# erincatto/solver2d

Measured on NVIDIA B200. Metric: constraint_iters_per_sec, higher is better.
Workload: dtype f32

## Files before the change

include/s2b_device.h:

```cpp
#pragma once

#include <stddef.h>
#include <stdint.h>

#ifdef __cplusplus
extern "C"
{
#endif

typedef struct s2bWorld s2bWorld;

#if defined(__GNUC__)
	#define S2B_API __attribute__((visibility("default")))
#else
	#define S2B_API
#endif


#define S2B_ROW_VALID 0x1
#define S2B_BODY_ADD_FORCE 0x8

typedef struct s2bBodyRow
{
	int32_t index;
// ... 104 lines not shown
};

typedef struct s2bCounters
{
	int32_t bodyCapacity, shapeCapacity, jointCapacity;
	int32_t contactCount;
	int32_t constraintCount;
	int32_t jointCount;
	int32_t groupCount;
	int32_t overflowCount;
	int32_t treeHeight;
	int32_t movedCount;
	int32_t pairPassCount;
	int32_t kernelLaunches;
	int32_t graphReplays;
	int32_t graphCaptures;
	int64_t scratchBytes;
	int32_t regionCount;
	int32_t cutCount;
	int32_t cutGroupCount;
	int32_t recolouredCount;
	int32_t largeLeafCount;
	int32_t pairRebuildCount;
} s2bCounters;


S2B_API s2bWorld* s2b_world_create(int cudaDevice, int solverType);
S2B_API void s2b_world_destroy(s2bWorld* world);

S2B_API void s2b_set_gravity(s2bWorld* world, float gx, float gy);
S2B_API void s2b_set_schedule(s2bWorld* world, int schedule);
S2B_API void s2b_set_max_colors(s2bWorld* world, int maxColors);
S2B_API void s2b_set_persistent(s2bWorld* world, int enable);
S2B_API void s2b_set_warm_gather(s2bWorld* world, int enable);
S2B_API void s2b_set_graph(s2bWorld* world, int enable);
S2B_API void s2b_set_regions(s2bWorld* world, int mode);
S2B_API void s2b_set_dataflow(s2bWorld* world, int enable);


S2B_API void s2b_upload_bodies(s2bWorld* world, const s2bBodyRow* rows, int count, int bodyCapacity);
S2B_API void s2b_upload_shapes(s2bWorld* world, const s2bShapeRow* rows, int count, int shapeCapacity);
S2B_API void s2b_upload_joints(s2bWorld* world, const s2bJointRow* rows, int count, int jointCapacity);
S2B_API void s2b_upload_contacts(s2bWorld* world, const s2bContactRow* rows, int count);
S2B_API void s2b_upload_joint_pairs(s2bWorld* world, const uint64_t* blockKeys, int blockCount, const uint64_t* destroyKeys,
									int destroyCount);
typedef struct s2bForceRow
// ... 57 lines not shown
```

solver2d_b200/csrc/device/broadphase.cu:

```cuda
#include "s2b_internal.cuh"

#include <cub/cub.cuh>
#include <thrust/iterator/counting_iterator.h>

#include <algorithm>

struct BroadScratch
{
	DevArray<int> validFlag;
	DevArray<int> leafShape;
	DevArray<unsigned> mortonIn, mortonOut;
	DevArray<int> leafIn, leafOut;
	DevArray<int> sortedShape;
	DevArray<int> counters;
	DevArray<int> boundsBits;
	DevArray<float4> nodeBox;
	DevArray<int> movedShapes;
	DevArray<int> movedFlag;
	DevArray<int> largeShapes;
	DevArray<unsigned long long> newKey;
	DevArray<int2> newShapes;
	DevArray<int> keepFlag, keepSlots;
	DevArray<unsigned long long> mergeKeyIn, mergeKeyOut;
	DevArray<int> mergeSrcIn, mergeSrcOut;
	DevArray<char> cubTemp;
	int newPairCap = 0;
	bool treeValid = false;
	int treeShapeCap = 0;
	int treeReuses = 0;
	DevArray<unsigned long long> pairHash;
	unsigned long long hashMask = 0;
	unsigned long long hashVersion = ~0ull;
	bool prefetched = false;
	bool lastPassRan = false;
	bool searchTimed = false;
	unsigned long long prefetchEpoch = 0, searchedVersion = 0;
	int searchedCount = 0;
	size_t prefetchTempBytes = 0;
	cudaEvent_t evSearch[2] = {nullptr, nullptr};
	cudaEvent_t searchDone = nullptr;
};

// ... 17 lines not shown
	}
	b->validFlag.release();
	b->leafShape.release();
	b->mortonIn.release();
	b->mortonOut.release();
	b->leafIn.release();
	b->leafOut.release();
	b->sortedShape.release();
	b->counters.release();
	b->boundsBits.release();
	b->nodeBox.release();
	b->movedShapes.release();
	b->movedFlag.release();
	b->newKey.release();
	b->newShapes.release();
	b->keepFlag.release();
	b->keepSlots.release();
	b->mergeKeyIn.release();
	b->mergeKeyOut.release();
	b->mergeSrcIn.release();
	b->mergeSrcOut.release();
	b->cubTemp.release();
	b->largeShapes.release();
	b->pairHash.release();
	for (int i = 0; i < 2; ++i)
	{
		if (b->evSearch[i] != nullptr)
		{
			cudaEventDestroy(b->evSearch[i]);
		}
	}
	if (b->searchDone != nullptr)
	{
		cudaEventDestroy(b->searchDone);
	}
	delete b;
	w->broad = nullptr;
}

enum
{
	BC_LEAVES = 0,
	BC_LARGE_LEAVES = 1,
	BC_NEW_PAIRS = 2,
	BC_KEPT = 3,
	BC_MOVED = 4,
	BC_HEIGHT = 5,
	BC_LARGE = 6,
	BC_REFIT_DONE = 7,
	BC_SIZE = 8
};


__device__ __forceinline__ int s2bFloatToOrdered(float f)
{
	int i = __float_as_int(f);
	return i >= 0 ? i : i ^ 0x7FFFFFFF;
}

__device__ __forceinline__ float s2bOrderedToFloat(int i)
{
	return __int_as_float(i >= 0 ? i : i ^ 0x7FFFFFFF);
}

__device__ __forceinline__ unsigned s2bExpandBits(unsigned v)
{
	v &= 0xFFFFu;
	v = (v | (v << 8)) & 0x00FF00FFu;
	v = (v | (v << 4)) & 0x0F0F0F0Fu;
	v = (v | (v << 2)) & 0x33333333u;
	v = (v | (v << 1)) & 0x55555555u;
	return v;
}
// ... 276 lines not shown
	__syncthreads();
	if (threadIdx.x == 0)
	{
		int total = 0;
		int warps = (blockDim.x + 31) >> 5;
		for (int k = 0; k < warps; ++k)
		{
			int c = warpOffset[k];
			warpOffset[k] = total;
			total += c;
		}
		blockBase = total > 0 ? atomicAdd(count, total) : 0;
	}
	__syncthreads();
	if (take)
	{
		list[blockBase + warpOffset[warp] + __popc(takers & ((1u << lane) - 1u))] = value;
	}
}

#define S2B_MAX_LARGE_MOVERS 64

__global__ void __launch_bounds__(256) s2bRefit(ShapeView s, const int* sortedShape, int* counters, const int* boundsBits,
												 float4* nodeBox, int* movedShapes, int* largeShapes)
{
	int n = counters[BC_LEAVES];
	int nh = n - min(counters[BC_LARGE_LEAVES], S2B_MAX_LARGE_LEAVES);
	int k = blockIdx.x * blockDim.x + threadIdx.x;
	bool moved = false;
	int shape = -1;
	float4 box = s2bEmptyBox();
	if (k < n)
	{
		shape = sortedShape[k];
		box = s.fat[shape];
		nodeBox[k] = box;
		moved = (s.head[shape].x & S2B_SHAPE_MOVED) != 0;
		if (moved && n >= 256)
		{
			float sceneArea = (s2bOrderedToFloat(boundsBits[6]) - s2bOrderedToFloat(boundsBits[4])) *
							  (s2bOrderedToFloat(boundsBits[7]) - s2bOrderedToFloat(boundsBits[5]));
			float area = (box.z - box.x) * (box.w - box.y);
			if (area * 256.0f > sceneArea)
			{
				int slot = atomicAdd(counters + BC_LARGE, 1);
				if (slot < S2B_MAX_LARGE_MOVERS)
				{
					largeShapes[slot] = shape;
					moved = false;
				}
			}
		}
	}
	s2bBlockAppend(moved, shape, movedShapes, counters + BC_MOVED);

	int offset[S2B_MAX_LEVELS], count[S2B_MAX_LEVELS];
	int top = s2bLevels(n, nh, offset, count);
	__shared__ float4 level1[256 / S2B_FANOUT];
	__shared__ bool lastBlock;
	float4 group = s2bUnion16(k < nh ? box : s2bEmptyBox());
	if ((threadIdx.x & (S2B_FANOUT - 1)) == 0)
	{
		if (top >= 1 && k < nh)
		{
			nodeBox[offset[1] + k / S2B_FANOUT] = group;
		}
		level1[threadIdx.x / S2B_FANOUT] = group;
	}
	__syncthreads();
	if (threadIdx.x < 32)
	{
		float4 node = s2bUnion16(threadIdx.x < 256 / S2B_FANOUT ? level1[threadIdx.x] : s2bEmptyBox());
		if (threadIdx.x == 0 && top >= 2 && blockIdx.x * 256 < nh)
		{
			nodeBox[offset[2] + blockIdx.x] = node;
// ... 18 lines not shown
			int first = i * S2B_FANOUT, last = min(first + S2B_FANOUT, count[l - 1]);
			float4 r = s2bEmptyBox();
			for (int j = first; j < last; ++j)
			{
				r = s2bUnion(r, __ldcg(below + j));
			}
			nodeBox[offset[l] + i] = r;
		}
		__syncthreads();
	}
	if (threadIdx.x == 0)
	{
		counters[BC_HEIGHT] = top + 1;
	}
}

struct PairQuery
{
	int shapeQ, bodyQ, keyQ;
	unsigned typeBodyQ;
	int4 headQ, filterQ;
};

__device__ __forceinline__ void s2bConsiderPair(const PairQuery& q, int other, const ShapeView& s, const BodyView& b, int* counters,
												 const unsigned long long* pairHash, unsigned long long hashMask,
												 const unsigned long long* jointKeys, int jointKeyCount, unsigned long long* newKey,
												 int2* newShapes, int newCap)
{
	int shapeQ = q.shapeQ;
	if (other == shapeQ)
	{
		return;
	}
	int4 headO = s.head[other];
	int bodyO = headO.y;
	int keyO = headO.z;
	unsigned typeBodyO = S2B_BODY_TYPE((unsigned)b.flags[bodyO]);
	if (q.typeBodyQ == S2B_BODY_KINEMATIC && typeBodyO != S2B_BODY_DYNAMIC)
	{
		return;
	}
	if ((headO.x & S2B_SHAPE_MOVED) && keyO > q.keyQ)
	{
		bool otherSeesUs = !(typeBodyO == S2B_BODY_KINEMATIC && q.typeBodyQ != S2B_BODY_DYNAMIC) && typeBodyO != S2B_BODY_STATIC;
		if (otherSeesUs)
		{
			return;
		}
	}
	if (bodyO == q.bodyQ)
	{
		return;
	}
	unsigned long long lo = (unsigned long long)(other < shapeQ ? other : shapeQ);
	unsigned long long hi = (unsigned long long)(other < shapeQ ? shapeQ : other);
	unsigned long long pairKey = (lo << 32) | hi;
	bool recreated = ((q.headQ.x | headO.x) & S2B_SHAPE_FRESH) != 0;
	if (recreated == false && s2bPairInHash(pairHash, hashMask, pairKey))
	{
		return;
	}
	int shapeA, shapeB;
	if (keyO < q.keyQ)
	{
		shapeA = other;
		shapeB = shapeQ;
	}
	else
	{
		shapeA = shapeQ;
		shapeB = other;
	}
	int4 filterO = s.filter[other];
	if (s2bShouldShapesCollide(shapeA == shapeQ ? q.filterQ : filterO, shapeA == shapeQ ? filterO : q.filterQ) == false)
	{
		return;
	}
	if (s2bJointOverride(jointKeys, jointKeyCount, q.bodyQ, bodyO))
	{
		return;
	}
	int typeA = ((shapeA == shapeQ ? q.headQ.x : headO.x) >> 1) & 0x7;
	int typeB = ((shapeA == shapeQ ? headO.x : q.headQ.x) >> 1) & 0x7;
	int kind = s2bPairKind(typeA, typeB);
	if (kind == 0)
	{
		return;
	}
	if (kind == 2)
	{
		int tmp = shapeA;
		shapeA = shapeB;
		shapeB = tmp;
	}
	int slot = atomicAdd(counters + BC_NEW_PAIRS, 1);
	if (slot < newCap)
	{
		newKey[slot] = pairKey;
		newShapes[slot] = make_int2(shapeA, shapeB);
	}
}

__device__ __forceinline__ bool s2bMakeQuery(PairQuery& q, int shapeQ, const ShapeView& s, const BodyView& b)
{
	q.shapeQ = shapeQ;
	q.headQ = s.head[shapeQ];
	q.filterQ = s.filter[shapeQ];
	q.bodyQ = q.headQ.y;
	q.keyQ = q.headQ.z;
	q.typeBodyQ = S2B_BODY_TYPE((unsigned)b.flags[q.bodyQ]);
	return q.typeBodyQ != S2B_BODY_STATIC;
}

#define S2B_QUERY_BATCH 16

__device__ __forceinline__ unsigned s2bOverlapMask(const float4* __restrict__ boxes, int count, float4 q)
{
	unsigned mask = 0;
#pragma unroll
	for (int j = 0; j < S2B_FANOUT; ++j)
	{
		if (j < count && s2bBoxesOverlap(q, __ldg(boxes + j)))
		{
			mask |= 1u << j;
		}
	}
	return mask;
}

__device__ __forceinline__ void s2bCollectKeptContacts(int i, const ContactView& c, int contactCount, const ShapeView& s,
														const unsigned long long* jointKeys, int jointKeyCount, int* keepSlots, int* counters)
{
	bool keep = false;
	if (i < contactCount)
	{
		int2 sh = c.shapes[i];
		int4 ha = s.head[sh.x], hb = s.head[sh.y];
		bool alive = (ha.x & S2B_ROW_VALID) && (hb.x & S2B_ROW_VALID) && (ha.x & S2B_SHAPE_FRESH) == 0 && (hb.x & S2B_SHAPE_FRESH) == 0;
		keep = alive && s2bBoxesOverlap(s.fat[sh.x], s.fat[sh.y]) && s2bJointOverride(jointKeys, jointKeyCount, ha.y, hb.y) == false;
	}
	s2bBlockAppend(keep, i, keepSlots, counters + BC_KEPT);
}

__global__ void __launch_bounds__(128) s2bFindPairs(ShapeView s, BodyView b, const int* sortedShape, int* counters, const int* movedShapes,
													const float4* __restrict__ nodeBox, int queryBlocks, ContactView cur, int contactCount,
													const unsigned long long* destroyKeys, int destroyKeyCount, int* keepSlots,
													const unsigned long long* pairHash, unsigned long long hashMask,
													const unsigned long long* jointKeys, int jointKeyCount, unsigned long long* newKey,
													int2* newShapes, int newCap)
{
	if ((int)blockIdx.x >= queryBlocks)
	{
		s2bCollectKeptContacts(((int)blockIdx.x - queryBlocks) * blockDim.x + threadIdx.x, cur, contactCount, s, destroyKeys,
							   destroyKeyCount, keepSlots, counters);
		return;
	}
	int n = counters[BC_LEAVES];
	int large = min(counters[BC_LARGE_LEAVES], S2B_MAX_LARGE_LEAVES);
	int nh = n - large;
	int movedCount = counters[BC_MOVED];
	int qi = blockIdx.x * blockDim.x + threadIdx.x;
	if (qi >= movedCount)
	{
		return;
	}
	PairQuery q;
	if (s2bMakeQuery(q, movedShapes[qi], s, b) == false)
	{
		return;
	}
	float4 boxQ = s.fat[q.shapeQ];

	int offset[S2B_MAX_LEVELS], count[S2B_MAX_LEVELS];
	int top = s2bLevels(n, nh, offset, count);
	unsigned pending[S2B_MAX_LEVELS];
	int base[S2B_MAX_LEVELS];
	int found[S2B_QUERY_BATCH + S2B_FANOUT];
	int nFound = 0;
	int level = top;
	bool walking = nh > 0;
	if (walking)
	{
		pending[top] = s2bOverlapMask(nodeBox + offset[top], count[top], boxQ);
		base[top] = 0;
	}
	while (walking || nFound > 0)
	{
		while (walking && nFound < S2B_QUERY_BATCH)
		{
			unsigned m = pending[level];
			if (level == 0 || m == 0)
			{
				for (; m != 0; m &= m - 1)
				{
					found[nFound++] = base[0] + __ffs(m) - 1;
				}
				level += 1;
				walking = level <= top;
				continue;
			}
			pending[level] = m & (m - 1);
			int first = (base[level] + __ffs(m) - 1) * S2B_FANOUT;
			pending[level - 1] = s2bOverlapMask(nodeBox + offset[level - 1] + first, min(S2B_FANOUT, count[level - 1] - first), boxQ);
			base[level - 1] = first;
			level -= 1;
		}
		for (int k = 0; k < nFound; ++k)
		{
			s2bConsiderPair(q, sortedShape[found[k]], s, b, counters, pairHash, hashMask, jointKeys, jointKeyCount, newKey, newShapes,
							newCap);
		}
		nFound = 0;
	}
	for (int i = nh; i < n; ++i)
	{
		if (s2bBoxesOverlap(boxQ, nodeBox[i]))
		{
			s2bConsiderPair(q, sortedShape[i], s, b, counters, pairHash, hashMask, jointKeys, jointKeyCount, newKey, newShapes, newCap);
		}
	}
}

__global__ void s2bFindPairsLarge(ShapeView s, BodyView b, const int* leafShape, int* counters, const int* largeShapes,
								  const unsigned long long* pairHash, unsigned long long hashMask, const unsigned long long* jointKeys,
								  int jointKeyCount, unsigned long long* newKey, int2* newShapes, int newCap)
{
	int n = counters[BC_LEAVES];
	int large = min(counters[BC_LARGE], S2B_MAX_LARGE_MOVERS);
	int k = blockIdx.x * blockDim.x + threadIdx.x;
	if (k >= n || large == 0)
	{
		return;
	}
	int other = leafShape[k];
	float4 boxO = s.fat[other];
	for (int i = 0; i < large; ++i)
	{
		int shapeQ = largeShapes[i];
		if (s2bBoxesOverlap(s.fat[shapeQ], boxO) == false)
		{
			continue;
		}
		PairQuery q;
		if (s2bMakeQuery(q, shapeQ, s, b))
		{
			s2bConsiderPair(q, other, s, b, counters, pairHash, hashMask, jointKeys, jointKeyCount, newKey, newShapes, newCap);
		}
	}
}

__device__ __forceinline__ unsigned long long s2bSqueezeKey(unsigned long long pairKey, int shapeBits)
{
	return ((pairKey >> 32) << shapeBits) | (pairKey & 0xFFFFFFFFull);
}

__global__ void s2bMergeKeys(const int* counters, const int* keepSlots, const unsigned long long* oldKeys,
							 const unsigned long long* newKey, unsigned long long* mergeKey, int* mergeSrc, int capacity, int shapeBits)
{
	int kept = counters[BC_KEPT], fresh = counters[BC_NEW_PAIRS];
	int t = blockIdx.x * blockDim.x + threadIdx.x;
	if (t >= capacity)
	{
		return;
	}
	if (t < kept)
	{
		mergeKey[t] = s2bSqueezeKey(oldKeys[keepSlots[t]], shapeBits);
		mergeSrc[t] = keepSlots[t];
	}
// ... 80 lines not shown


#define MAIL_BC_BASE 16

static size_t bpReserve(s2bWorld* w, BroadScratch* B)
{
	cudaStream_t st = w->stream;
	int shapeCap = w->shapeCap;
	int oldCount = w->contactCount;
	size_t nS = (size_t)shapeCap;
	B->validFlag.reserve(nS, st, false);
	B->leafShape.reserve(nS, st, false);
	B->mortonIn.reserve(nS, st, false);
	B->mortonOut.reserve(nS, st, false);
	B->leafIn.reserve(nS, st, false);
	B->leafOut.reserve(nS, st, false);
	B->sortedShape.reserve(nS, st, false);
	B->counters.reserve(BC_SIZE, st, false);
	B->boundsBits.reserve(8, st, false);
	B->nodeBox.reserve(nS + nS / 8 + 64, st, false);
	B->movedShapes.reserve(nS, st, false);
	B->movedFlag.reserve(nS, st, false);
	B->largeShapes.reserve(S2B_MAX_LARGE_MOVERS, st, false);
	B->keepFlag.reserve((size_t)std::max(oldCount, 1), st, false);
	B->keepSlots.reserve((size_t)std::max(oldCount, 1), st, false);
	if (B->newPairCap == 0)
	{
		B->newPairCap = 8 * shapeCap + 1024;
	}
	size_t need = 0, tempBytes = 0;
	cub::DeviceSelect::Flagged(nullptr, need, thrust::counting_iterator<int>(0), (int*)nullptr, (int*)nullptr, (int*)nullptr,
							   std::max(shapeCap, oldCount), st);
	tempBytes = std::max(tempBytes, need);
	cub::DeviceRadixSort::SortPairs(nullptr, need, (unsigned*)nullptr, (unsigned*)nullptr, (int*)nullptr, (int*)nullptr, shapeCap, 0,
									32, st);
	tempBytes = std::max(tempBytes, need);
	B->newKey.reserve((size_t)B->newPairCap, st, false);
	B->newShapes.reserve((size_t)B->newPairCap, st, false);
	B->cubTemp.reserve(tempBytes + 256, st, false, false);
	return tempBytes;
}

static void bpSearch(s2bWorld* w, BroadScratch* B)
{
	cudaStream_t st = w->stream;
	int shapeCap = w->shapeCap;
// ... 16 lines not shown
		S2B_LAUNCH(w, s2bFlagValidShapes, gridFor(shapeCap, 256), 256, 0, sv, B->validFlag.p);
		size_t tb = B->cubTemp.cap;
		cub::DeviceSelect::Flagged(B->cubTemp.p, tb, thrust::counting_iterator<int>(0), B->validFlag.p, B->leafShape.p,
								   B->counters.p + BC_LEAVES, shapeCap, st);
		w->kernelLaunches += 2;

		const int lo = 0x7F7FFFFF, hi = (int)0x80800000;
		int initBounds[8] = {lo, lo, hi, hi, lo, lo, hi, hi};
		S2B_CHECK(cudaMemcpyAsync(B->boundsBits.p, initBounds, sizeof(initBounds), cudaMemcpyHostToDevice, st));
		S2B_LAUNCH(w, s2bSceneBounds, gridFor(shapeCap, 256), 256, 0, sv, B->leafShape.p, B->counters.p, B->boundsBits.p);
		S2B_LAUNCH(w, s2bMortonCodes, gridFor(shapeCap, 256), 256, 0, sv, B->leafShape.p, B->counters.p, B->boundsBits.p,
				   B->mortonIn.p, B->leafIn.p, shapeCap);
		tb = B->cubTemp.cap;
		cub::DeviceRadixSort::SortPairs(B->cubTemp.p, tb, B->mortonIn.p, B->mortonOut.p, B->leafIn.p, B->leafOut.p, shapeCap, 0, 32, st);
		w->kernelLaunches += 5;
		S2B_LAUNCH(w, s2bSortedShapes, gridFor(shapeCap, 256), 256, 0, B->leafShape.p, B->leafOut.p, B->counters.p, B->sortedShape.p);
		B->treeValid = true;
		B->treeShapeCap = shapeCap;
		B->treeReuses = 0;
		w->pairRebuildCount += 1;
	}

	S2B_LAUNCH(w, s2bRefit, gridFor(shapeCap, 256), 256, 0, sv, B->sortedShape.p, B->counters.p, B->boundsBits.p, B->nodeBox.p,
			   B->movedShapes.p, B->largeShapes.p);

	if (B->hashVersion != w->contactTableVersion || B->pairHash.p == nullptr)
	{
		unsigned long long size = 1024;
		while (size < 2ull * (unsigned long long)std::max(oldCount, 1))
		{
			size <<= 1;
		}
		B->pairHash.reserve((size_t)size, st, false, false);
		B->hashMask = size - 1;
		S2B_CHECK(cudaMemsetAsync(B->pairHash.p, 0xFF, sizeof(unsigned long long) * (size_t)size, st));
		if (oldCount > 0)
		{
			S2B_LAUNCH(w, s2bBuildPairHash, gridFor(oldCount, 256), 256, 0, cur.key.p, oldCount, B->pairHash.p, B->hashMask);
		}
		B->hashVersion = w->contactTableVersion;
	}

	int queryBlocks = gridFor(shapeCap, 128);
	S2B_LAUNCH(w, s2bFindPairs, queryBlocks + (oldCount > 0 ? gridFor(oldCount, 128) : 0), 128, 0, sv, bv, B->sortedShape.p,
			   B->counters.p, B->movedShapes.p, B->nodeBox.p, queryBlocks, makeView(cur), oldCount, w->jointDestroyKeys.p,
			   w->jointDestroyCount, B->keepSlots.p, B->pairHash.p, B->hashMask, w->jointPairKeys.p, w->jointPairCount, B->newKey.p,
			   B->newShapes.p, newCap);
	S2B_LAUNCH(w, s2bFindPairsLarge, gridFor(shapeCap, 256), 256, 0, sv, bv, B->leafShape.p, B->counters.p, B->largeShapes.p,
			   B->pairHash.p, B->hashMask, w->jointPairKeys.p, w->jointPairCount, B->newKey.p, B->newShapes.p, newCap);
	S2B_CHECK(cudaMemcpyAsync(w->hostMail + MAIL_BC_BASE, B->counters.p, sizeof(int) * BC_SIZE, cudaMemcpyDeviceToHost, st));
	B->searchedCount = oldCount;
	B->searchedVersion = w->contactTableVersion;
}

static void bpCommit(s2bWorld* w, BroadScratch* B, int fresh, int kept, size_t tempBytes)
{
	cudaStream_t st = w->stream;
	int shapeCap = w->shapeCap;
	int oldCount = w->contactCount;
	ShapeView sv = shapeView(w);
	ContactColumns& cur = w->contacts[w->cur];
	ContactColumns& nxt = w->contacts[w->cur ^ 1];
	int total = kept + fresh;
	if (fresh == 0 && kept == oldCount)
	{
	}
	else
	{
		nxt.reserve((size_t)std::max(total, 1), st, w->sticky, false);
		if (total > 0)
		{
			size_t need = 0;
			B->mergeKeyIn.reserve((size_t)total, st, false);
			B->mergeKeyOut.reserve((size_t)total, st, false);
			B->mergeSrcIn.reserve((size_t)total, st, false);
// ... 75 lines not shown
	return ms;
}

void s2bBroadphaseUpdatePairs(s2bWorld* w)
{
	S2bEpochFreeze freeze;
	cudaStream_t st = w->stream;
	BroadScratch* B = getBroad(w);
	w->dMovedFlag.reserve(4, st, true);

	if (B->prefetched)
	{
		B->prefetched = false;
		bool valid = w->pairsDirty == false && B->prefetchEpoch == w->uploadEpoch && B->searchedVersion == w->contactTableVersion &&
					 B->searchedCount == w->contactCount && w->prefetchPairs == 1;
		if (valid)
		{
			S2B_CHECK(cudaEventSynchronize(B->searchDone));
			S2B_CHECK(cudaEventRecord(w->timer.ev[0], st));
			const int* hc = w->hostMail + MAIL_BC_BASE;
			int fresh = hc[BC_NEW_PAIRS], kept = hc[BC_KEPT];
			if (fresh <= B->newPairCap)
			{
				w->treeHeight = hc[BC_HEIGHT];
				w->largeLeafCount = std::min(hc[BC_LARGE_LEAVES], S2B_MAX_LARGE_LEAVES);
				B->lastPassRan = hc[BC_MOVED] > 0 || hc[BC_LARGE] > 0;
				bpCommit(w, B, fresh, kept, B->prefetchTempBytes);
				return;
			}
			B->newPairCap = fresh + fresh / 2 + 1024;
		}
	}

	bool run = w->pairsDirty;
	if (run == false)
	{
		if (w->movedEvent != nullptr)
		{
			S2B_CHECK(cudaEventSynchronize(w->movedEvent));
		}
		else
		{
			S2B_CHECK(cudaStreamSynchronize(st));
		}
		run = w->hostMail[MAIL_MOVED] > 0;
	}
	S2B_CHECK(cudaEventRecord(w->timer.ev[0], st));
	B->lastPassRan = run && w->shapeCap > 0;
	if (run == false || w->shapeCap == 0)
	{
		return;
	}

	for (int attempt = 0; attempt < 4; ++attempt)
	{
		size_t tempBytes = bpReserve(w, B);
		bpSearch(w, B);
		S2B_CHECK(cudaStreamSynchronize(st));
		const int* hc = w->hostMail + MAIL_BC_BASE;
		int fresh = hc[BC_NEW_PAIRS], kept = hc[BC_KEPT];
		if (fresh > B->newPairCap)
		{
			B->newPairCap = fresh + fresh / 2 + 1024;
			continue;
		}
		w->treeHeight = hc[BC_HEIGHT];
		w->largeLeafCount = std::min(hc[BC_LARGE_LEAVES], S2B_MAX_LARGE_LEAVES);
		bpCommit(w, B, fresh, kept, tempBytes);
		break;
	}
}
```

solver2d_b200/csrc/device/s2b_internal.cuh:

```cuda
#pragma once

#include "s2b_device.h"
#include "solver2d/constants.h"
#include "solver2d/aabb.h"
#include "solver2d/math.h"

#include <cuda_runtime.h>
#include <stdint.h>
#include <stdio.h>
#include <stdlib.h>
#include <string.h>
#include <vector>

#define S2B_CHECK(call)                                                                                                \
	do                                                                                                                 \
	{                                                                                                                  \
		cudaError_t err__ = (call);                                                                                    \
		if (err__ != cudaSuccess)                                                                                      \
		{                                                                                                              \
			fprintf(stderr, "solver2d-b200: CUDA error %s at %s:%d (%s) — no CPU fallback, aborting\n",                 \
					cudaGetErrorString(err__), __FILE__, __LINE__, #call);                                             \
			abort();                                                                                                   \
		}                                                                                                              \
	} while (0)
// ... 281 lines not shown
	DevArray<unsigned long long> jointDestroyKeys;
	int jointDestroyCount = 0;

	float* hostState = nullptr;
	void* bulkHost[2] = {nullptr, nullptr};
	size_t bulkBytes[2] = {0, 0};
	cudaEvent_t bulkEvent[2] = {nullptr, nullptr};
	int bulkNext = 0, bulkCurrent = 0;
	DevArray<char> dBulk;
	float* hostXf = nullptr;
	size_t hostXfFloats = 0;
	DevArray<float4> dXf;
	size_t hostStateFloats = 0;
	DevArray<float4> dState;

	ContactColumns contacts[2];
	int cur = 0;
	int contactCount = 0;
	bool sticky = false;

	bool pairsDirty = true;
	unsigned long long uploadEpoch = 0;
	int prefetchPairs = 1;
	int kempe = 1;
	int wholeIslandBodies = 1200;
	int residentRegions = 1;
	int hubDegree = 48;
	int fusePositions = 1;
	int kempeGrid = 0;
	DevArray<int> dMovedFlag;
	int pairPassCount = 0;
	int treeHeight = 0;
	int largeLeafCount = 0;
	int pairRebuildCount = 0;

	std::vector<unsigned long long> orderHint;

	struct SolverScratch* scratch = nullptr;
	struct BroadScratch* broad = nullptr;

	int* hostMail = nullptr;
	int* devMail = nullptr;

	int kernelLaunches = 0;
	DevArray<unsigned long long> dWork;
	cudaEvent_t solveKernelStart = nullptr, solveKernelEnd = nullptr;
	bool solveKernelTimed = false;
	cudaEvent_t markEvents[2] = {nullptr, nullptr};
	cudaEvent_t movedEvent = nullptr;
	cudaStream_t copyStream = nullptr;
	unsigned long long xfSeq = 0, finalizeSeq = ~0ull;
	int sideCopies = 1;
	StageTimer timer;
	float stageMs[4] = {0, 0, 0, 0};

	DevArray<char> l2Flush;
};
// ... 82 lines not shown
```

solver2d_b200/csrc/device/solver.cu:

```cuda
#include "persistent.cuh"

#include <cooperative_groups.h>
#include <cuda/barrier>
#include <cub/cub.cuh>
#include <thrust/iterator/counting_iterator.h>

#include <algorithm>

namespace cg = cooperative_groups;


SolverScratch* s2bGetSolverScratch(s2bWorld* w)
{
	if (w->scratch == nullptr)
	{
		w->scratch = new SolverScratch();
	}
	return w->scratch;
}

void s2bFreeSolverScratch(s2bWorld* w)
{
	SolverScratch* s = w->scratch;
	if (s == nullptr)
// ... 3334 lines not shown
		out->cutCount = w->scratch->regions > 0 ? counts[CNT_CUT] : 0;
		out->regionCount = counts[CNT_REGIONS_ON] != 0 ? w->scratch->regions : 0;
		out->overflowCount = counts[CNT_OVERFLOW_C] + counts[CNT_OVERFLOW_J];
		if (w->scratch->kempeState.p != nullptr)
		{
			int ks[4];
			S2B_CHECK(cudaMemcpy(ks, w->scratch->kempeState.p, sizeof(ks), cudaMemcpyDeviceToHost));
			out->recolouredCount = ks[KS_FIXED];
		}
		if (w->scratch->bodyTicket.p != nullptr && w->scratch->flowErrorOffset > 0)
		{
			int flag = 0;
			S2B_CHECK(cudaMemcpy(&flag, w->scratch->bodyTicket.p + w->scratch->flowErrorOffset, sizeof(int), cudaMemcpyDeviceToHost));
			if (flag != 0)
			{
				fprintf(stderr, "solver2d-b200: a ticketed solver pass ran into its spin limit (internal error)\n");
				abort();
			}
		}
	}
	out->treeHeight = w->treeHeight;
	out->largeLeafCount = w->largeLeafCount;
	out->pairRebuildCount = w->pairRebuildCount;
	out->movedCount = w->hostMail[MAIL_MOVED];
	out->pairPassCount = w->pairPassCount;
	out->kernelLaunches = w->kernelLaunches;
	out->graphReplays = w->scratch != nullptr ? w->scratch->graphReplays : 0;
	out->graphCaptures = w->scratch != nullptr ? w->scratch->graphCaptures : 0;
}

extern "C" void s2b_set_solve_trace(s2bWorld* w, int capacity)
{
	s2bGetSolverScratch(w)->traceCap = capacity > 0 ? capacity + 1 : 0;
}

extern "C" int s2b_get_solve_trace(s2bWorld* w, uint64_t* out, int maxEntries)
{
	S2B_CHECK(cudaSetDevice(w->device));
	S2B_CHECK(cudaStreamSynchronize(w->stream));
	SolverScratch* s = s2bGetSolverScratch(w);
	if (s->trace.p == nullptr || s->traceCap == 0)
	{
		return 0;
	}
	unsigned long long n = 0;
	S2B_CHECK(cudaMemcpy(&n, s->trace.p, sizeof(n), cudaMemcpyDeviceToHost));
// ... 78 lines not shown
```

solver2d_b200/csrc/device/world.cu:

```cuda
#include "s2b_internal.cuh"


__global__ void s2bScatterBodies(const s2bBodyRow* __restrict__ rows, int count, BodyView b, int* schedDirty)
{
	int t = blockIdx.x * blockDim.x + threadIdx.x;
	if (t >= count)
	{
		return;
	}
	s2bBodyRow r = rows[t];
	int i = r.index;
	{
		bool wasValid = (b.flags[i] & S2B_BODY_VALID) != 0, isValid = (r.flags & S2B_BODY_VALID) != 0;
		bool wasMovable = b.vel[i].w != 0.0f || b.prm[i].w != 0.0f, isMovable = r.invMass != 0.0f || r.invI != 0.0f;
		if (wasValid != isValid || (isValid && wasMovable != isMovable))
		{
			*schedDirty = 1;
		}
	}
	b.vel[i] = make_float4(r.linearVelocity[0], r.linearVelocity[1], r.angularVelocity, r.invMass);
	b.pose[i] = make_float4(0.0f, 0.0f, r.rot[0], r.rot[1]);
	b.pos[i] = make_float4(r.position[0], r.position[1], r.invI, r.I);
	b.org[i] = make_float4(r.origin[0], r.origin[1], r.localCenter[0], r.localCenter[1]);
	if (r.flags & S2B_BODY_ADD_FORCE)
// ... 282 lines not shown
	}
	w->device = cudaDevice;
	S2B_CHECK(cudaSetDevice(cudaDevice));
	S2B_CHECK(cudaStreamCreateWithFlags(&w->stream, cudaStreamNonBlocking));
	cudaDeviceProp prop;
	S2B_CHECK(cudaGetDeviceProperties(&prop, cudaDevice));
	w->smCount = prop.multiProcessorCount;
	w->coopSupported = prop.cooperativeLaunch;
	{
		const char* env = getenv("S2B_WARM_GATHER");
		if (env != nullptr)
		{
			w->gatherWarm = atoi(env) != 0 ? 1 : 0;
		}
		env = getenv("S2B_GRAPH");
		if (env != nullptr)
		{
			w->useGraph = atoi(env) != 0 ? 1 : 0;
		}
		env = getenv("S2B_PREFETCH_PAIRS");
		if (env != nullptr)
		{
			w->prefetchPairs = atoi(env);
		}
		env = getenv("S2B_FUSE_POSITIONS");
		if (env != nullptr)
		{
			w->fusePositions = atoi(env);
		}
		env = getenv("S2B_HUB_DEGREE");
		if (env != nullptr)
		{
			w->hubDegree = atoi(env);
		}
		env = getenv("S2B_RESIDENT");
		if (env != nullptr)
		{
			w->residentRegions = atoi(env);
		}
		env = getenv("S2B_SIDE_COPIES");
		if (env != nullptr)
		{
			w->sideCopies = atoi(env);
		}
		env = getenv("S2B_WHOLE_ISLAND");
		if (env != nullptr)
// ... 842 lines not shown
```

solver2d_b200/device.py:

```python
from __future__ import annotations

import ctypes as C
import os

import numpy as np

HERE = os.path.dirname(os.path.abspath(__file__))
LIB_PATH = os.path.join(HERE, "libsolver2d.so")

BODY_ROW = np.dtype([
    ("index", "<i4"), ("flags", "<i4"), ("origin", "<f4", 2), ("position", "<f4", 2), ("rot", "<f4", 2),
    ("linearVelocity", "<f4", 2), ("angularVelocity", "<f4"), ("localCenter", "<f4", 2), ("mass", "<f4"),
    ("invMass", "<f4"), ("I", "<f4"), ("invI", "<f4"), ("force", "<f4", 2), ("torque", "<f4"),
    ("linearDamping", "<f4"), ("angularDamping", "<f4"), ("gravityScale", "<f4"),
], align=True)

SHAPE_ROW = np.dtype([
    ("index", "<i4"), ("flags", "<i4"), ("body", "<i4"), ("proxyKey", "<i4"), ("categoryBits", "<u4"),
    ("maskBits", "<u4"), ("groupIndex", "<i4"), ("friction", "<f4"), ("aabb", "<f4", 4), ("fatAABB", "<f4", 4),
    ("radius", "<f4"), ("count", "<i4"), ("vertices", "<f4", 16), ("normals", "<f4", 16),
], align=True)

JOINT_ROW = np.dtype([
    ("index", "<i4"), ("flags", "<i4"), ("bodyA", "<i4"), ("bodyB", "<i4"), ("localOriginAnchorA", "<f4", 2),
# ... 7 lines not shown
    ("tangentImpulse", "<f4"), ("frictionAnchorA", "<f4", 2), ("frictionAnchorB", "<f4", 2),
    ("frictionNormalA", "<f4", 2), ("frictionNormalB", "<f4", 2), ("id", "<i4"), ("persisted", "<i4"),
], align=True)

CONTACT_ROW = np.dtype([
    ("shapeA", "<i4"), ("shapeB", "<i4"), ("bodyA", "<i4"), ("bodyB", "<i4"), ("pointCount", "<i4"),
    ("frictionPersisted", "<i4"), ("friction", "<f4"), ("normal", "<f4", 2), ("points", CONTACT_POINT, 2),
    ("cacheCount", "<i4"), ("cacheIndexA", "u1", 4), ("cacheIndexB", "u1", 4), ("cacheMetric", "<f4"),
], align=True)


class StepContext(C.Structure):
    _fields_ = [("dt", C.c_float), ("inv_dt", C.c_float), ("h", C.c_float), ("inv_h", C.c_float),
                ("iterations", C.c_int32), ("extraIterations", C.c_int32), ("warmStart", C.c_int32)]


class Counters(C.Structure):
    _fields_ = [("bodyCapacity", C.c_int32), ("shapeCapacity", C.c_int32), ("jointCapacity", C.c_int32),
                ("contactCount", C.c_int32), ("constraintCount", C.c_int32), ("jointCount", C.c_int32),
                ("groupCount", C.c_int32), ("overflowCount", C.c_int32), ("treeHeight", C.c_int32),
                ("movedCount", C.c_int32), ("pairPassCount", C.c_int32), ("kernelLaunches", C.c_int32),
                ("graphReplays", C.c_int32), ("graphCaptures", C.c_int32), ("scratchBytes", C.c_int64),
                ("regionCount", C.c_int32), ("cutCount", C.c_int32), ("cutGroupCount", C.c_int32), ("recolouredCount", C.c_int32),
                ("largeLeafCount", C.c_int32), ("pairRebuildCount", C.c_int32)]


SCHEDULE_COLOR, SCHEDULE_WAVEFRONT = 0, 1
ROW_VALID = 0x1
SHAPE_MOVED = 0x10
JOINT_ENABLE_LIMIT, JOINT_ENABLE_MOTOR, JOINT_COLLIDE_CONNECTED = 0x10, 0x20, 0x40

ABI_SYMBOLS = [
    "s2b_world_create", "s2b_world_destroy", "s2b_set_gravity", "s2b_set_schedule", "s2b_set_max_colors",
    "s2b_set_persistent", "s2b_upload_bodies", "s2b_upload_shapes", "s2b_upload_joints", "s2b_upload_contacts",
    "s2b_upload_joint_pairs", "s2b_mark_pairs_dirty", "s2b_set_contact_order", "s2b_update_pairs",
    "s2b_update_contacts", "s2b_solve", "s2b_finalize", "s2b_step", "s2b_sync", "s2b_download_bodies",
    "s2b_download_all_bodies", "s2b_download_shape_boxes", "s2b_download_joints", "s2b_download_contacts",
    "s2b_download_solve_order", "s2b_download_islands", "s2b_prefetch_pairs", "s2b_get_counters", "s2b_pack_body_state", "s2b_timed_steps", "s2b_last_stage_ms",
    "s2b_flush_l2", "s2b_time_color_kernel", "s2b_version", "s2b_abi_sizes", "s2b_upload_forces", "s2b_host_alloc",
    "s2b_host_free", "s2b_sync_body_state", "s2b_set_warm_gather", "s2b_eval_atan2", "s2b_set_dataflow", "s2b_set_regions", "s2b_set_graph", "s2b_get_stream", "s2b_add_forces", "s2b_download_transforms",
]


def make_context(solver: str, dt: float, vel_iters: int, pos_iters: int, warm_start: bool = True) -> StepContext:
    from .capi import SUBSTEPPING
    f = np.float32
    ctx = StepContext()
# ... 215 lines not shown
```

Before: 5.825 billion.

## Group broadphase pair queries per half-warp with shared candidate lists

Adds a cooperative query mode in which each half-warp of 16 spatially sorted moved leaves walks the BVH once using the union of their boxes. Overlapping leaves are collected into shared-memory candidate lists, and each lane then tests its own box against them. Hits are compacted warp-wide before pair filtering. Groups that overflow the stack or candidate buffers fall back to the old per-lane traversal. The aim is to cut divergent per-thread tree walks and redundant node loads, at the cost of more shared memory, warp syncs, extra atomics for counters, and wasted tests when grouped boxes are spread apart.

New measurement: 5.690 billion (median of 6 runs). 2.3% lower.

```diff
diff --git a/include/s2b_device.h b/include/s2b_device.h
--- a/include/s2b_device.h
+++ b/include/s2b_device.h
@@ -150,6 +150,9 @@
 	int32_t recolouredCount;
 	int32_t largeLeafCount;
 	int32_t pairRebuildCount;
+	int32_t pairQueryFallbacks;
+	int64_t pairQueryGroups;
+	int64_t pairQueryCandidates;
 } s2bCounters;
 
 
diff --git a/solver2d_b200/csrc/device/broadphase.cu b/solver2d_b200/csrc/device/broadphase.cu
--- a/solver2d_b200/csrc/device/broadphase.cu
+++ b/solver2d_b200/csrc/device/broadphase.cu
@@ -18,6 +18,7 @@
 	DevArray<int> movedShapes;
 	DevArray<int> movedFlag;
 	DevArray<int> largeShapes;
+	DevArray<unsigned char> queryFlag;
 	DevArray<unsigned long long> newKey;
 	DevArray<int2> newShapes;
 	DevArray<int> keepFlag, keepSlots;
@@ -81,6 +82,7 @@
 	b->mergeSrcOut.release();
 	b->cubTemp.release();
 	b->largeShapes.release();
+	b->queryFlag.release();
 	b->pairHash.release();
 	for (int i = 0; i < 2; ++i)
 	{
@@ -107,7 +109,10 @@
 	BC_HEIGHT = 5,
 	BC_LARGE = 6,
 	BC_REFIT_DONE = 7,
-	BC_SIZE = 8
+	BC_QUERY_GROUPS = 8,
+	BC_FALLBACK_GROUPS = 9,
+	BC_CANDIDATES = 10,
+	BC_SIZE = 11
 };
 
 
@@ -430,7 +435,7 @@
 #define S2B_MAX_LARGE_MOVERS 64
 
 __global__ void __launch_bounds__(256) s2bRefit(ShapeView s, const int* sortedShape, int* counters, const int* boundsBits,
-												 float4* nodeBox, int* movedShapes, int* largeShapes)
+												 float4* nodeBox, int* movedShapes, int* largeShapes, unsigned char* queryFlag)
 {
 	int n = counters[BC_LEAVES];
 	int nh = n - min(counters[BC_LARGE_LEAVES], S2B_MAX_LARGE_LEAVES);
@@ -459,6 +464,7 @@
 				}
 			}
 		}
+		queryFlag[k] = moved ? 1 : 0;
 	}
 	s2bBlockAppend(moved, shape, movedShapes, counters + BC_MOVED);
 
@@ -523,11 +529,25 @@
 	int4 headQ, filterQ;
 };
 
-__device__ __forceinline__ void s2bConsiderPair(const PairQuery& q, int other, const ShapeView& s, const BodyView& b, int* counters,
-												 const unsigned long long* pairHash, unsigned long long hashMask,
-												 const unsigned long long* jointKeys, int jointKeyCount, unsigned long long* newKey,
-												 int2* newShapes, int newCap)
-{
+struct PairRules
+{
+	ShapeView s;
+	BodyView b;
+	const int* sortedShape;
+	int* counters;
+	const unsigned long long* pairHash;
+	unsigned long long hashMask;
+	const unsigned long long* jointKeys;
+	int jointKeyCount;
+	unsigned long long* newKey;
+	int2* newShapes;
+	int newCap;
+};
+
+__device__ __forceinline__ void s2bConsiderPair(const PairQuery& q, int other, const PairRules& r)
+{
+	const ShapeView& s = r.s;
+	const BodyView& b = r.b;
 	int shapeQ = q.shapeQ;
 	if (other == shapeQ)
 	{
@@ -557,7 +577,7 @@
 	unsigned long long hi = (unsigned long long)(other < shapeQ ? shapeQ : other);
 	unsigned long long pairKey = (lo << 32) | hi;
 	bool recreated = ((q.headQ.x | headO.x) & S2B_SHAPE_FRESH) != 0;
-	if (recreated == false && s2bPairInHash(pairHash, hashMask, pairKey))
+	if (recreated == false && s2bPairInHash(r.pairHash, r.hashMask, pairKey))
 	{
 		return;
 	}
@@ -577,7 +597,7 @@
 	{
 		return;
 	}
-	if (s2bJointOverride(jointKeys, jointKeyCount, q.bodyQ, bodyO))
+	if (s2bJointOverride(r.jointKeys, r.jointKeyCount, q.bodyQ, bodyO))
 	{
 		return;
 	}
@@ -594,11 +614,11 @@
 		shapeA = shapeB;
 		shapeB = tmp;
 	}
-	int slot = atomicAdd(counters + BC_NEW_PAIRS, 1);
-	if (slot < newCap)
-	{
-		newKey[slot] = pairKey;
-		newShapes[slot] = make_int2(shapeA, shapeB);
+	int slot = atomicAdd(r.counters + BC_NEW_PAIRS, 1);
+	if (slot < r.newCap)
+	{
+		r.newKey[slot] = pairKey;
+		r.newShapes[slot] = make_int2(shapeA, shapeB);
 	}
 }
 
@@ -643,35 +663,9 @@
 	s2bBlockAppend(keep, i, keepSlots, counters + BC_KEPT);
 }
 
-__global__ void __launch_bounds__(128) s2bFindPairs(ShapeView s, BodyView b, const int* sortedShape, int* counters, const int* movedShapes,
-													const float4* __restrict__ nodeBox, int queryBlocks, ContactView cur, int contactCount,
-													const unsigned long long* destroyKeys, int destroyKeyCount, int* keepSlots,
-													const unsigned long long* pairHash, unsigned long long hashMask,
-													const unsigned long long* jointKeys, int jointKeyCount, unsigned long long* newKey,
-													int2* newShapes, int newCap)
-{
-	if ((int)blockIdx.x >= queryBlocks)
-	{
-		s2bCollectKeptContacts(((int)blockIdx.x - queryBlocks) * blockDim.x + threadIdx.x, cur, contactCount, s, destroyKeys,
-							   destroyKeyCount, keepSlots, counters);
-		return;
-	}
-	int n = counters[BC_LEAVES];
-	int large = min(counters[BC_LARGE_LEAVES], S2B_MAX_LARGE_LEAVES);
-	int nh = n - large;
-	int movedCount = counters[BC_MOVED];
-	int qi = blockIdx.x * blockDim.x + threadIdx.x;
-	if (qi >= movedCount)
-	{
-		return;
-	}
-	PairQuery q;
-	if (s2bMakeQuery(q, movedShapes[qi], s, b) == false)
-	{
-		return;
-	}
-	float4 boxQ = s.fat[q.shapeQ];
-
+__device__ void s2bLaneQuery(const PairQuery& q, float4 boxQ, int n, int nh, const float4* __restrict__ nodeBox,
+							 const PairRules& r)
+{
 	int offset[S2B_MAX_LEVELS], count[S2B_MAX_LEVELS];
 	int top = s2bLevels(n, nh, offset, count);
 	unsigned pending[S2B_MAX_LEVELS];
@@ -708,8 +702,7 @@
 		}
 		for (int k = 0; k < nFound; ++k)
 		{
-			s2bConsiderPair(q, sortedShape[found[k]], s, b, counters, pairHash, hashMask, jointKeys, jointKeyCount, newKey, newShapes,
-							newCap);
+			s2bConsiderPair(q, r.sortedShape[found[k]], r);
 		}
 		nFound = 0;
 	}
@@ -717,17 +710,209 @@
 	{
 		if (s2bBoxesOverlap(boxQ, nodeBox[i]))
 		{
-			s2bConsiderPair(q, sortedShape[i], s, b, counters, pairHash, hashMask, jointKeys, jointKeyCount, newKey, newShapes, newCap);
-		}
-	}
-}
-
-__global__ void s2bFindPairsLarge(ShapeView s, BodyView b, const int* leafShape, int* counters, const int* largeShapes,
-								  const unsigned long long* pairHash, unsigned long long hashMask, const unsigned long long* jointKeys,
-								  int jointKeyCount, unsigned long long* newKey, int2* newShapes, int newCap)
-{
-	int n = counters[BC_LEAVES];
-	int large = min(counters[BC_LARGE], S2B_MAX_LARGE_MOVERS);
+			s2bConsiderPair(q, r.sortedShape[i], r);
+		}
+	}
+}
+
+#define S2B_QUERY_WARPS (128 / 32)
+#define S2B_GROUP_CANDIDATES 128
+#define S2B_GROUP_STACK 64
+#define S2B_GROUP_HITS 64
+
+struct GroupQueryShared
+{
+	float4 candBox[2][S2B_GROUP_CANDIDATES];
+	int candSlot[2][S2B_GROUP_CANDIDATES];
+	PairQuery query[32];
+	int2 hits[S2B_GROUP_HITS];
+	unsigned stack[2][S2B_GROUP_STACK];
+	int levelOffset[S2B_MAX_LEVELS], levelCount[S2B_MAX_LEVELS];
+};
+
+__device__ __forceinline__ void s2bGroupHit(bool hit, int leaf, int& nHits, GroupQueryShared& g, const PairRules& r)
+{
+	int lane = threadIdx.x & 31;
+	unsigned m = __ballot_sync(0xFFFFFFFFu, hit);
+	if (hit)
+	{
+		g.hits[nHits + __popc(m & ((1u << lane) - 1u))] = make_int2(lane, leaf);
+	}
+	nHits += __popc(m);
+	if (nHits >= 32)
+	{
+		__syncwarp();
+		int2 h = g.hits[lane];
+		int rest = nHits - 32;
+		int2 later = lane < rest ? g.hits[32 + lane] : h;
+		__syncwarp();
+		if (lane < rest)
+		{
+			g.hits[lane] = later;
+		}
+		nHits = rest;
+		PairQuery q = g.query[h.x];
+		s2bConsiderPair(q, r.sortedShape[h.y], r);
+	}
+}
+
+__device__ __forceinline__ void s2bGroupQuery(const float4* __restrict__ nodeBox, const unsigned char* queryFlag, int n, int nh,
+											  const PairRules& r)
+{
+	__shared__ GroupQueryShared shared[S2B_QUERY_WARPS];
+	GroupQueryShared& g = shared[threadIdx.x >> 5];
+	int lane = threadIdx.x & 31;
+	int leaf = blockIdx.x * blockDim.x + threadIdx.x;
+	PairQuery q;
+	bool active = leaf < n && queryFlag[leaf] != 0 && s2bMakeQuery(q, r.sortedShape[leaf], r.s, r.b);
+	if (__ballot_sync(0xFFFFFFFFu, active) == 0)
+	{
+		return;
+	}
+	float4 boxQ = active ? nodeBox[leaf] : s2bEmptyBox();
+	bool inGroup = active && leaf < nh && !(isnan(boxQ.x) || isnan(boxQ.y) || isnan(boxQ.z) || isnan(boxQ.w));
+	bool alone = active && !inGroup;
+	unsigned grouped = __ballot_sync(0xFFFFFFFFu, inGroup);
+	if (grouped != 0)
+	{
+		int half = lane >> 4;
+		unsigned halfLanes = 0xFFFFu << (16 * half), below = (1u << lane) - 1u;
+		float4 u = inGroup ? boxQ : s2bEmptyBox();
+		u = s2bUnion16(u);
+		if (inGroup)
+		{
+			g.query[lane] = q;
+		}
+		if (lane == 0)
+		{
+			int top = s2bLevels(n, nh, g.levelOffset, g.levelCount);
+			g.stack[0][0] = g.stack[1][0] = (unsigned)(top + 1) << 28;
+		}
+		__syncwarp();
+
+		int depth = (grouped & halfLanes) != 0 ? 1 : 0, nCand = 0;
+		bool overflow = false;
+		while (__any_sync(0xFFFFFFFFu, depth > 0 && !overflow))
+		{
+			bool walking = depth > 0 && !overflow;
+			float4 box = s2bEmptyBox();
+			bool hit = false;
+			int childLevel = 0, child = 0;
+			if (walking)
+			{
+				unsigned entry = g.stack[half][depth - 1];
+				childLevel = (int)(entry >> 28) - 1;
+				child = (int)(entry & 0x0FFFFFFFu) * S2B_FANOUT + (lane & (S2B_FANOUT - 1));
+				if (child < g.levelCount[childLevel])
+				{
+					box = __ldg(nodeBox + g.levelOffset[childLevel] + child);
+					hit = s2bBoxesOverlap(u, box);
+				}
+			}
+			__syncwarp();
+			depth -= walking ? 1 : 0;
+			unsigned leaves = __ballot_sync(0xFFFFFFFFu, hit && childLevel == 0) & halfLanes;
+			unsigned nodes = __ballot_sync(0xFFFFFFFFu, hit && childLevel > 0) & halfLanes;
+			if (hit)
+			{
+				if (childLevel == 0)
+				{
+					int at = nCand + __popc(leaves & below);
+					if (at < S2B_GROUP_CANDIDATES)
+					{
+						g.candBox[half][at] = box;
+						g.candSlot[half][at] = child;
+					}
+				}
+				else
+				{
+					int at = depth + __popc(nodes & below);
+					if (at < S2B_GROUP_STACK)
+					{
+						g.stack[half][at] = ((unsigned)childLevel << 28) | (unsigned)child;
+					}
+				}
+			}
+			nCand += __popc(leaves);
+			depth += __popc(nodes);
+			overflow = overflow || nCand > S2B_GROUP_CANDIDATES || depth > S2B_GROUP_STACK;
+			__syncwarp();
+		}
+		if ((lane & 15) == 0 && (grouped & halfLanes) != 0)
+		{
+			atomicAdd(r.counters + BC_QUERY_GROUPS, 1);
+			atomicAdd(r.counters + (overflow ? BC_FALLBACK_GROUPS : BC_CANDIDATES), overflow ? 1 : nCand);
+		}
+		if (overflow)
+		{
+			alone = alone || inGroup;
+			inGroup = false;
+			nCand = 0;
+		}
+		int rounds = max(__shfl_sync(0xFFFFFFFFu, nCand, 0), __shfl_sync(0xFFFFFFFFu, nCand, 16));
+		int nHits = 0;
+		for (int c = 0; c < rounds; ++c)
+		{
+			bool mine = inGroup && c < nCand;
+			s2bGroupHit(mine && s2bBoxesOverlap(boxQ, g.candBox[half][c]), mine ? g.candSlot[half][c] : 0, nHits, g, r);
+		}
+		if (__any_sync(0xFFFFFFFFu, inGroup))
+		{
+			for (int i = nh; i < n; ++i)
+			{
+				s2bGroupHit(inGroup && s2bBoxesOverlap(boxQ, nodeBox[i]), i, nHits, g, r);
+			}
+		}
+		__syncwarp();
+		if (lane < nHits)
+		{
+			int2 h = g.hits[lane];
+			PairQuery hq = g.query[h.x];
+			s2bConsiderPair(hq, r.sortedShape[h.y], r);
+		}
+	}
+	if (alone)
+	{
+		s2bLaneQuery(q, boxQ, n, nh, nodeBox, r);
+	}
+}
+
+__global__ void __launch_bounds__(128) s2bFindPairs(PairRules r, const int* movedShapes, const unsigned char* queryFlag, int groupQuery,
+													const float4* __restrict__ nodeBox, int queryBlocks, ContactView cur, int contactCount,
+													const unsigned long long* destroyKeys, int destroyKeyCount, int* keepSlots)
+{
+	if ((int)blockIdx.x >= queryBlocks)
+	{
+		s2bCollectKeptContacts(((int)blockIdx.x - queryBlocks) * blockDim.x + threadIdx.x, cur, contactCount, r.s, destroyKeys,
+							   destroyKeyCount, keepSlots, r.counters);
+		return;
+	}
+	int n = r.counters[BC_LEAVES];
+	int large = min(r.counters[BC_LARGE_LEAVES], S2B_MAX_LARGE_LEAVES);
+	int nh = n - large;
+	if (groupQuery)
+	{
+		s2bGroupQuery(nodeBox, queryFlag, n, nh, r);
+		return;
+	}
+	int qi = blockIdx.x * blockDim.x + threadIdx.x;
+	if (qi >= r.counters[BC_MOVED])
+	{
+		return;
+	}
+	PairQuery q;
+	if (s2bMakeQuery(q, movedShapes[qi], r.s, r.b) == false)
+	{
+		return;
+	}
+	s2bLaneQuery(q, r.s.fat[q.shapeQ], n, nh, nodeBox, r);
+}
+
+__global__ void s2bFindPairsLarge(PairRules r, const int* leafShape, const int* largeShapes)
+{
+	const ShapeView& s = r.s;
+	int n = r.counters[BC_LEAVES];
+	int large = min(r.counters[BC_LARGE], S2B_MAX_LARGE_MOVERS);
 	int k = blockIdx.x * blockDim.x + threadIdx.x;
 	if (k >= n || large == 0)
 	{
@@ -743,9 +928,9 @@
 			continue;
 		}
 		PairQuery q;
-		if (s2bMakeQuery(q, shapeQ, s, b))
-		{
-			s2bConsiderPair(q, other, s, b, counters, pairHash, hashMask, jointKeys, jointKeyCount, newKey, newShapes, newCap);
+		if (s2bMakeQuery(q, shapeQ, s, r.b))
+		{
+			s2bConsiderPair(q, other, r);
 		}
 	}
 }
@@ -872,6 +1057,7 @@
 	B->movedShapes.reserve(nS, st, false);
 	B->movedFlag.reserve(nS, st, false);
 	B->largeShapes.reserve(S2B_MAX_LARGE_MOVERS, st, false);
+	B->queryFlag.reserve(nS, st, false);
 	B->keepFlag.reserve((size_t)std::max(oldCount, 1), st, false);
 	B->keepSlots.reserve((size_t)std::max(oldCount, 1), st, false);
 	if (B->newPairCap == 0)
@@ -934,7 +1120,7 @@
 	}
 
 	S2B_LAUNCH(w, s2bRefit, gridFor(shapeCap, 256), 256, 0, sv, B->sortedShape.p, B->counters.p, B->boundsBits.p, B->nodeBox.p,
-			   B->movedShapes.p, B->largeShapes.p);
+			   B->movedShapes.p, B->largeShapes.p, B->queryFlag.p);
 
 	if (B->hashVersion != w->contactTableVersion || B->pairHash.p == nullptr)
 	{
@@ -953,16 +1139,25 @@
 		B->hashVersion = w->contactTableVersion;
 	}
 
+	PairRules rules = {sv, bv, B->sortedShape.p, B->counters.p, B->pairHash.p, B->hashMask, w->jointPairKeys.p, w->jointPairCount,
+					   B->newKey.p, B->newShapes.p, newCap};
 	int queryBlocks = gridFor(shapeCap, 128);
-	S2B_LAUNCH(w, s2bFindPairs, queryBlocks + (oldCount > 0 ? gridFor(oldCount, 128) : 0), 128, 0, sv, bv, B->sortedShape.p,
-			   B->counters.p, B->movedShapes.p, B->nodeBox.p, queryBlocks, makeView(cur), oldCount, w->jointDestroyKeys.p,
-			   w->jointDestroyCount, B->keepSlots.p, B->pairHash.p, B->hashMask, w->jointPairKeys.p, w->jointPairCount, B->newKey.p,
-			   B->newShapes.p, newCap);
-	S2B_LAUNCH(w, s2bFindPairsLarge, gridFor(shapeCap, 256), 256, 0, sv, bv, B->leafShape.p, B->counters.p, B->largeShapes.p,
-			   B->pairHash.p, B->hashMask, w->jointPairKeys.p, w->jointPairCount, B->newKey.p, B->newShapes.p, newCap);
+	S2B_LAUNCH(w, s2bFindPairs, queryBlocks + (oldCount > 0 ? gridFor(oldCount, 128) : 0), 128, 0, rules,
+			   B->movedShapes.p, B->queryFlag.p, w->pairQueryGroup, B->nodeBox.p, queryBlocks, makeView(cur), oldCount,
+			   w->jointDestroyKeys.p, w->jointDestroyCount, B->keepSlots.p);
+	S2B_LAUNCH(w, s2bFindPairsLarge, gridFor(shapeCap, 256), 256, 0, rules, B->leafShape.p, B->largeShapes.p);
 	S2B_CHECK(cudaMemcpyAsync(w->hostMail + MAIL_BC_BASE, B->counters.p, sizeof(int) * BC_SIZE, cudaMemcpyDeviceToHost, st));
 	B->searchedCount = oldCount;
 	B->searchedVersion = w->contactTableVersion;
+}
+
+static void bpReadCounters(s2bWorld* w, const int* hc)
+{
+	w->treeHeight = hc[BC_HEIGHT];
+	w->largeLeafCount = std::min(hc[BC_LARGE_LEAVES], S2B_MAX_LARGE_LEAVES);
+	w->pairQueryFallbacks += hc[BC_FALLBACK_GROUPS];
+	w->pairQueryGroups += hc[BC_QUERY_GROUPS];
+	w->pairQueryCandidates += hc[BC_CANDIDATES];
 }
 
 static void bpCommit(s2bWorld* w, BroadScratch* B, int fresh, int kept, size_t tempBytes)
@@ -1084,8 +1279,7 @@
 			int fresh = hc[BC_NEW_PAIRS], kept = hc[BC_KEPT];
 			if (fresh <= B->newPairCap)
 			{
-				w->treeHeight = hc[BC_HEIGHT];
-				w->largeLeafCount = std::min(hc[BC_LARGE_LEAVES], S2B_MAX_LARGE_LEAVES);
+				bpReadCounters(w, hc);
 				B->lastPassRan = hc[BC_MOVED] > 0 || hc[BC_LARGE] > 0;
 				bpCommit(w, B, fresh, kept, B->prefetchTempBytes);
 				return;
@@ -1126,8 +1320,7 @@
 			B->newPairCap = fresh + fresh / 2 + 1024;
 			continue;
 		}
-		w->treeHeight = hc[BC_HEIGHT];
-		w->largeLeafCount = std::min(hc[BC_LARGE_LEAVES], S2B_MAX_LARGE_LEAVES);
+		bpReadCounters(w, hc);
 		bpCommit(w, B, fresh, kept, tempBytes);
 		break;
 	}
diff --git a/solver2d_b200/csrc/device/s2b_internal.cuh b/solver2d_b200/csrc/device/s2b_internal.cuh
--- a/solver2d_b200/csrc/device/s2b_internal.cuh
+++ b/solver2d_b200/csrc/device/s2b_internal.cuh
@@ -327,6 +327,7 @@
 	bool pairsDirty = true;
 	unsigned long long uploadEpoch = 0;
 	int prefetchPairs = 1;
+	int pairQueryGroup = 1;
 	int kempe = 1;
 	int wholeIslandBodies = 1200;
 	int residentRegions = 1;
@@ -338,6 +339,9 @@
 	int treeHeight = 0;
 	int largeLeafCount = 0;
 	int pairRebuildCount = 0;
+	int pairQueryFallbacks = 0;
+	long long pairQueryGroups = 0;
+	long long pairQueryCandidates = 0;
 
 	std::vector<unsigned long long> orderHint;
 
diff --git a/solver2d_b200/csrc/device/solver.cu b/solver2d_b200/csrc/device/solver.cu
--- a/solver2d_b200/csrc/device/solver.cu
+++ b/solver2d_b200/csrc/device/solver.cu
@@ -3380,6 +3380,9 @@
 	out->treeHeight = w->treeHeight;
 	out->largeLeafCount = w->largeLeafCount;
 	out->pairRebuildCount = w->pairRebuildCount;
+	out->pairQueryFallbacks = w->pairQueryFallbacks;
+	out->pairQueryGroups = w->pairQueryGroups;
+	out->pairQueryCandidates = w->pairQueryCandidates;
 	out->movedCount = w->hostMail[MAIL_MOVED];
 	out->pairPassCount = w->pairPassCount;
 	out->kernelLaunches = w->kernelLaunches;
diff --git a/solver2d_b200/csrc/device/world.cu b/solver2d_b200/csrc/device/world.cu
--- a/solver2d_b200/csrc/device/world.cu
+++ b/solver2d_b200/csrc/device/world.cu
@@ -328,6 +328,11 @@
 		if (env != nullptr)
 		{
 			w->prefetchPairs = atoi(env);
+		}
+		env = getenv("S2B_PAIR_QUERY");
+		if (env != nullptr)
+		{
+			w->pairQueryGroup = strcmp(env, "lane") == 0 ? 0 : 1;
 		}
 		env = getenv("S2B_FUSE_POSITIONS");
 		if (env != nullptr)
diff --git a/solver2d_b200/device.py b/solver2d_b200/device.py
--- a/solver2d_b200/device.py
+++ b/solver2d_b200/device.py
@@ -53,7 +53,8 @@
                 ("movedCount", C.c_int32), ("pairPassCount", C.c_int32), ("kernelLaunches", C.c_int32),
                 ("graphReplays", C.c_int32), ("graphCaptures", C.c_int32), ("scratchBytes", C.c_int64),
                 ("regionCount", C.c_int32), ("cutCount", C.c_int32), ("cutGroupCount", C.c_int32), ("recolouredCount", C.c_int32),
-                ("largeLeafCount", C.c_int32), ("pairRebuildCount", C.c_int32)]
+                ("largeLeafCount", C.c_int32), ("pairRebuildCount", C.c_int32), ("pairQueryFallbacks", C.c_int32),
+                ("pairQueryGroups", C.c_int64), ("pairQueryCandidates", C.c_int64)]
 
 
 SCHEDULE_COLOR, SCHEDULE_WAVEFRONT = 0, 1
```
